# DarylFernandes99/custom-yolo-implmentation

Hardware: AMD Instinct MI355X
Metric: images/sec (640x640 bf16) (higher is better)
Workload: dtype bf16; 1 GPU; preset s (width 32..512, depth 1) 640x640 train step (fwd+DFL/QFL loss+bwd+grad sync+AdamW), COCO-80 synthetic, 32 img/GPU; global_batch=32, parallelism=dp1, hip_graph=True, optimizer_in_graph=True, deterministic_mode=False

## Files before the change

custom-yolo-implmentation_amd/csrc/conv_generic.hip:

```cpp
#include "conv_host.h"

namespace {

template <typename T, int V, bool ACC>
__global__ void k_conv_generic(ConvGeom g, const T* __restrict__ src, const T* __restrict__ wm,
                               const float* __restrict__ bias, T* __restrict__ dst) {
    long total = (long)g.N * g.Hg * g.Wg * g.Cd;
    for (long i = blockIdx.x * (long)blockDim.x + threadIdx.x; i < total; i += (long)gridDim.x * blockDim.x) {
        int cd = (int)(i % g.Cd);
        long q = i / g.Cd;
        int b = (int)(q % g.Wg);
        long t2 = q / g.Wg;
        int a = (int)(t2 % g.Hg);
        long n = t2 / g.Hg;
        float acc = bias ? bias[cd] : 0.f;
        const T* wrow = wm + (long)cd * g.Kpad;
        for (int t = 0; t < g.ntaps; ++t) {
            int hs = a * g.sstride + g.dh[t], ws = b * g.sstride + g.dw[t];
            if (hs < 0 || hs >= g.Hs || ws < 0 || ws >= g.Ws) continue;
            const T* sp = src + ((n * g.Hs + hs) * g.Ws + ws) * (long)g.lds;
            const T* wp = wrow + t * g.Cs;
            for (int c = 0; c < g.Cs; c += V) {
                float xs[V], wv[V];
                load_pack<T, V>(sp + c, xs);
// ... 314 lines not shown
    if (!conv_supported(k, stride)) return 0;
    const int Kpad = round_up32(k * k * Cin);
    if (wgrad_path(x, ldx, dy, ldy, N, H, W, Cin, OH, OW, Cout, dtype, algo) == 2)
        return mfma_wgrad2_ws_elems(Kpad, N, H, W, Cin, OH, OW, Cout, k);
    return (long)Cout * Kpad;
}

int yolo_conv2d_wgrad(const void* x, int ldx, const void* dy, int ldy, float* ws, void* dw_oihw, int dw_dtype, int N,
                      int H, int W, int Cin, int OH, int OW, int Cout, int k, int stride, int dtype, int algo,
                      hipStream_t st) {
    if (!conv_supported(k, stride)) return YOLO_ERR_ARG;
    const int K = k * k * Cin, Kpad = round_up32(K);
    const int path = wgrad_path(x, ldx, dy, ldy, N, H, W, Cin, OH, OW, Cout, dtype, algo);
    if (path == 2)
        return mfma_wgrad2_launch(x, ldx, dy, ldy, ws, dw_oihw, dw_dtype, Kpad, N, H, W, Cin, OH, OW, Cout, k, stride, dtype, st);
    if (algo == 2) return YOLO_ERR_ARG;
    float* dwp = ws;
    int rc = yolo_zero_async(dwp, (size_t)Cout * Kpad * sizeof(float), st);
    if (rc) return rc;
    if (path == 3) {
        rc = mfma_wgrad_launch(x, ldx, dy, ldy, dwp, Kpad, N, H, W, Cin, OH, OW, Cout, k, stride, dtype, st);
    } else if (dtype == YOLO_F32 && f32_wgrad_eligible(x, ldx, dy, ldy, Cin, Cout)) {
        rc = f32_wgrad_launch((const float*)x, ldx, (const float*)dy, ldy, dwp, Kpad, N, H, W, Cin, OH, OW, Cout, k, stride, st);
    } else {
        long nrows = (long)N * OH;
        long elems = (long)Cout * K;
        int gx = (int)((elems + 255) / 256);
        long want_slabs = 4096 / (gx > 0 ? gx : 1);
        if (want_slabs < 1) want_slabs = 1;
        if (want_slabs > nrows) want_slabs = nrows;
        if (want_slabs < 1) want_slabs = 1;
        int rps = (int)((nrows + want_slabs - 1) / want_slabs);
        if (rps < 1) rps = 1;
        int gy = (int)((nrows + rps - 1) / rps);
        if (gy > 0)
            YOLO_DISPATCH_T(dtype, hipLaunchKernelGGL((k_wgrad_generic<T>), dim3(gx, gy), dim3(256), 0, st, (const T*)x, ldx,
                                                      (const T*)dy, ldy, dwp, Kpad, N, H, W, Cin, OH, OW, Cout, k, stride, rps));
        rc = YOLO_LAUNCH_CHECK();
    }
    if (rc) return rc;
    return yolo_conv_unpack_wgrad(dwp, Cout, Cin, k, dw_oihw, dw_dtype, st);
}

}

static dim3 dw_grid(int nrows, int cv) {
    int tpr = cv < 256 ? cv : 256;
    return dim3((unsigned)(nrows < 4096 ? nrows : 4096), (unsigned)ceil_div(cv, tpr));
}

template <bool FLIP>
static int dw_launch(const void* x, int ldx, const float* w, void* y, int ldy, int N, int H, int W, int C, int dtype,
                     int accumulate, hipStream_t st) {
    const int fast = dw_strip_launch(FLIP, x, ldx, w, y, ldy, N, H, W, C, dtype, accumulate, nullptr, st);
    if (fast >= 0) return fast;
    YOLO_DISPATCH_T(dtype, {
        if (vecok<T>(x, ldx, C) && vecok<T>(y, ldy, C)) {
            constexpr int V = vec_of<T>::N;
            hipLaunchKernelGGL((k_dw3x3<T, V, FLIP>), dw_grid(N * H, C / V), dim3(256), 0, st, (const T*)x, ldx, w, (T*)y,
                               ldy, N, H, W, C, accumulate);
        } else {
            hipLaunchKernelGGL((k_dw3x3<T, 1, FLIP>), dw_grid(N * H, C), dim3(256), 0, st, (const T*)x, ldx, w, (T*)y, ldy,
                               N, H, W, C, accumulate);
        }
    });
    return YOLO_LAUNCH_CHECK();
}

extern "C" {

int yolo_dwconv3x3_fwd(const void* x, int ldx, const float* w, void* y, int ldy, int N, int H, int W, int C, int dtype,
                       hipStream_t st) {
    return dw_launch<false>(x, ldx, w, y, ldy, N, H, W, C, dtype, 0, st);
}

int yolo_dwconv3x3_fwd_stats(const void* x, int ldx, const float* w, void* y, int ldy, float* stats, int N, int H, int W, int C,
                             int dtype, hipStream_t st) {
    const int fast = dw_strip_launch(false, x, ldx, w, y, ldy, N, H, W, C, dtype, 0, stats, st);
    return fast < 0 ? 1 : fast;
}

int yolo_dwconv3x3_fwd_act(const void* x, int ldx, const float* w, const float* bias, void* y, int ldy, int N, int H, int W, int C,
                           int act, int dtype, hipStream_t st) {
    if (bias == nullptr || (act != 0 && act != 1)) return YOLO_ERR_ARG;
    const int fast = dw_strip_launch(false, x, ldx, w, y, ldy, N, H, W, C, dtype, 0, nullptr, st, bias, act);
    return fast < 0 ? 1 : fast;
}

int yolo_dwconv3x3_dgrad(const void* dy, int lddy, const float* w, void* dx, int lddx, int N, int H, int W, int C,
                         int accumulate, int dtype, hipStream_t st) {
    return dw_launch<true>(dy, lddy, w, dx, lddx, N, H, W, C, dtype, accumulate, st);
}

int yolo_dw_wgrad_nslab(int N, int H) {
    int nrows = N * H;
    int slabs = nrows < 1024 ? nrows : 1024;
    int rps = (nrows + slabs - 1) / slabs;
    return (nrows + rps - 1) / rps;
}

int yolo_dwconv3x3_wgrad(const void* x, int ldx, const void* dy, int ldy, float* dw, float* partial, int N, int H,
                         int W, int C, int dtype, hipStream_t st) {
    int nrows = N * H;
    int slabs = yolo_dw_wgrad_nslab(N, H);
    int rps = (nrows + slabs - 1) / slabs;
    const int fast = dw_strip_wgrad_launch(x, ldx, dy, ldy, partial, slabs, N, H, W, C, dtype, st);
    if (fast > 0) return fast;
    if (fast < 0) YOLO_DISPATCH_T(dtype, {
        if (vecok<T>(x, ldx, C) && vecok<T>(dy, ldy, C)) {
            constexpr int V = vec_of<T>::N;
            int cv = C / V, tpr = cv < 256 ? cv : 256;
            hipLaunchKernelGGL((k_dw3x3_wgrad<T, V>), dim3(slabs, ceil_div(cv, tpr)), dim3(256), 0, st, (const T*)x, ldx,
                               (const T*)dy, ldy, partial, N, H, W, C, rps);
        } else {
            int tpr = C < 256 ? C : 256;
            hipLaunchKernelGGL((k_dw3x3_wgrad<T, 1>), dim3(slabs, ceil_div(C, tpr)), dim3(256), 0, st, (const T*)x, ldx,
                               (const T*)dy, ldy, partial, N, H, W, C, rps);
        }
    });
    hipLaunchKernelGGL(k_dw_wgrad_finalize, dim3(ceil_div(C * 9, 32)), dim3(1024), 0, st, partial, slabs, C * 9, dw);
    return YOLO_LAUNCH_CHECK();
}

}
```

custom-yolo-implmentation_amd/csrc/conv_host.h:

```cpp
#pragma once
#include "common.h"
#include "conv_geom.h"

enum ConvKind {
    CONV_NONE = -1,
    CONV_VALU = 0,
    CONV_GATHER = 1,
    CONV_HALO = 2,
    CONV_RING = 3,
    CONV_ROWS = 4,
    CONV_UP2 = 5
};
struct RingTile { int bm, bn, nst, bk; };
struct ConvChoice {
    int kind;
    int joint;
    int variant;
    int bn;
    RingTile ring;
};
ConvChoice conv_select(const ConvGeom* gs, int n, int cls, int dtype, const void* src, const void* wm, const void* dst, int algo);

ConvTune& conv_tune();
int conv_wide_flag();

int mfma_conv_addressable(const ConvGeom& g, int dtype, const void* src, const void* wm, const void* dst);

int valu_conv_launch(const ConvGeom& g, const void* src, const void* wm, const float* bias, void* dst, int accumulate, int dtype,
                     hipStream_t st);
int mfma_conv_eligible(const ConvGeom& g, int dtype, const void* src, const void* wm, const void* dst);
int mfma_conv_launch(const ConvGeom& g, int bn, const void* src, const void* wm, const float* bias, void* dst, int accumulate,
                     int dtype, hipStream_t st);
int halo_conv_eligible(const ConvGeom& g);
int halo_conv_launch(const ConvGeom& g, int variant, const void* src, const void* wm, const float* bias, void* dst,
                     int accumulate, int dtype, hipStream_t st);
int ring_conv_eligible(const ConvGeom& g, int dtype, const void* src, const void* wm, const void* dst);
int ring_conv_launch(const ConvGeom* gs, int n, const RingTile& t, const long* wm_off, long wm_elems, const void* src,
                     const void* wm, const float* bias, void* dst, int accumulate, int dtype, hipStream_t st);
int rows_conv_eligible(const ConvGeom& g);
int rows_conv_launch(const ConvGeom& g, int variant, const void* src, const void* wm, const float* bias, void* dst, int accumulate,
                     int dtype, hipStream_t st);
int up2_conv_eligible(const ConvGeom* gs, int dtype);
int up2_conv_launch(const ConvGeom* gs, int variant, const long* wm_off, long wm_elems, const void* src, const void* wm, void* dst,
                    int accumulate, int dtype, hipStream_t st);
int f32_conv_eligible(const ConvGeom& g, const void* src, const void* wm, const void* dst);
int f32_conv_launch(const ConvGeom& g, const float* src, const float* wm, const float* bias, float* dst, int accumulate,
                    hipStream_t st);

int f32_wgrad_eligible(const void* x, int ldx, const void* dy, int ldy, int Cin, int Cout);
int f32_wgrad_launch(const float* x, int ldx, const float* dy, int ldy, float* dwp, int Kpad, int N, int H, int W, int Cin,
                     int OH, int OW, int Cout, int k, int stride, hipStream_t st);
int mfma_wgrad_eligible(int Cin, int Cout, int ldx, int ldy, int dtype, const void* x, const void* dy);
int mfma_wgrad_launch(const void* x, int ldx, const void* dy, int ldy, float* dwp, int Kpad, int N, int H, int W,
                      int Cin, int OH, int OW, int Cout, int k, int stride, int dtype, hipStream_t st);
long mfma_wgrad2_plan(int Kpad, int N, int H, int W, int Cin, int OH, int OW, int Cout, int k);
long mfma_wgrad2_ws_elems(int Kpad, int N, int H, int W, int Cin, int OH, int OW, int Cout, int k);
int mfma_wgrad2_launch(const void* x, int ldx, const void* dy, int ldy, float* part, void* dw_oihw, int dw_dtype, int Kpad,
                       int N, int H, int W, int Cin, int OH, int OW, int Cout, int k, int stride, int dtype, hipStream_t st);

int dw_strip_launch(bool flip, const void* x, int ldx, const float* w, void* y, int ldy, int N, int H, int W, int C, int dtype,
                    int accumulate, float* stats, hipStream_t st, const float* bias = nullptr, int act = 0);
int dw_strip_wgrad_launch(const void* x, int ldx, const void* dy, int ldy, float* partial, int nslab, int N, int H, int W, int C,
                          int dtype, hipStream_t st);

extern "C" int yolo_bn_stats_acc(const void* y, int ldy, long npix, int C, int dtype, float* acc, hipStream_t st);
extern "C" int yolo_copy_channels(const void* src, int ld_src, void* dst, int ld_dst, long npix, int C, int accumulate, int dtype,
                                  hipStream_t st);

static inline bool conv_supported(int k, int stride) { return (k == 1 && stride == 1) || (k == 3 && (stride == 1 || stride == 2)); }
```

custom-yolo-implmentation_amd/csrc/dwconv.hip:

```cpp
#include "conv_host.h"

namespace {

typedef unsigned int u32x4 __attribute__((ext_vector_type(4)));
typedef _Float16 h16x2 __attribute__((ext_vector_type(2)));

template <typename T> __device__ __forceinline__ void unpack8(const u32x4& v, float (&o)[8]);
template <> __device__ __forceinline__ void unpack8<bf16_t>(const u32x4& v, float (&o)[8]) {
#pragma unroll
    for (int i = 0; i < 4; ++i) {
        o[2 * i] = __uint_as_float(v[i] << 16);
        o[2 * i + 1] = __uint_as_float(v[i] & 0xffff0000u);
    }
}
template <> __device__ __forceinline__ void unpack8<f16_t>(const u32x4& v, float (&o)[8]) {
#pragma unroll
    for (int i = 0; i < 4; ++i) {
        const unsigned int u = v[i];
        o[2 * i] = (float)__builtin_bit_cast(_Float16, (unsigned short)(u & 0xffffu));
        o[2 * i + 1] = (float)__builtin_bit_cast(_Float16, (unsigned short)(u >> 16));
    }
}

struct DwGeom {
    int N, H, W, C, ldx, ldy;
    int cvb;
    int ncol;
    int nsh;
    int ncb;
    long total;
    const float* bias;
    int act;
};

constexpr int OOB = (int)0x80000000;

template <bool FLIP>
__device__ __forceinline__ void stage_taps(float* wl, const float* __restrict__ w, int c0, int C, int cvb) {
    for (int i = threadIdx.x; i < cvb * 8 * 9; i += 256) {
        const int ch = i / 9, t = i - ch * 9;
        const float v = (c0 + ch < C) ? w[(long)(c0 + ch) * 9 + (FLIP ? 8 - t : t)] : 0.f;
        wl[((t * 2 + ((ch >> 2) & 1)) * cvb + (ch >> 3)) * 4 + (ch & 3)] = v;
    }
}

template <typename T, int R, bool FLIP>
__global__ __launch_bounds__(256) void k_dw3x3_strip(DwGeom g, const T* __restrict__ x, const float* __restrict__ w,
                                                     T* __restrict__ y, int accumulate, float* __restrict__ stats) {
    extern __shared__ __attribute__((aligned(16))) float wl[];
    const int c0 = blockIdx.y * g.cvb * 8;
    stage_taps<FLIP>(wl, w, c0, g.C, g.cvb);
    __syncthreads();
    const int cgl = threadIdx.x % g.cvb, col = threadIdx.x / g.cvb;
    const int ch = c0 + cgl * 8;
    const bool active = col < g.ncol && ch < g.C;
    float ssum[8], ssq[8];
#pragma unroll
    for (int j = 0; j < 8; ++j) ssum[j] = ssq[j] = 0.f;
    const __amdgpu_buffer_rsrc_t rs =
        __builtin_amdgcn_make_buffer_rsrc(const_cast<T*>(x), 0, g.N * g.H * g.W * g.ldx * 2, 0x00020000);
    const float4* wq = reinterpret_cast<const float4*>(wl) + cgl;
    for (long s = blockIdx.x; active && s < g.total; s += gridDim.x) {
        const int cbk = (int)(s % g.ncb);
        const long t2 = s / g.ncb;
        const int sh = (int)(t2 % g.nsh), n = (int)(t2 / g.nsh);
        const int h0 = sh * R, wc = cbk * g.ncol + col;
        if (wc >= g.W) continue;
        u32x4 v[R + 2][3];
#pragma unroll
        for (int r = 0; r < R + 2; ++r) {
            const int hs = h0 - 1 + r;
            const bool rok = (unsigned)hs < (unsigned)g.H;
#pragma unroll
            for (int c = 0; c < 3; ++c) {
                const int ws = wc - 1 + c;
                const bool ok = rok && (unsigned)ws < (unsigned)g.W;
                const int off = ok ? ((((n * g.H + hs) * g.W + ws) * g.ldx + ch) * 2) : OOB;
                v[r][c] = __builtin_amdgcn_raw_buffer_load_b128(rs, off, 0, 0);
            }
        }
        float acc[R][8];
#pragma unroll
        for (int o = 0; o < R; ++o)
#pragma unroll
            for (int j = 0; j < 8; ++j) acc[o][j] = 0.f;
#pragma unroll
        for (int r = 0; r < R + 2; ++r)
#pragma unroll
            for (int c = 0; c < 3; ++c) {
                float f[8];
                unpack8<T>(v[r][c], f);
#pragma unroll
                for (int kh = 0; kh < 3; ++kh) {
                    const int o = r - kh;
                    if (o < 0 || o >= R) continue;
// ... 78 lines not shown
            if (wc >= g.W) continue;
            u32x4 gv[R], v[R + 2][3];
#pragma unroll
            for (int o = 0; o < R; ++o) {
                const bool ok = h0 + o < g.H;
                gv[o] = __builtin_amdgcn_raw_buffer_load_b128(rsy, ok ? ((((n * g.H + h0 + o) * g.W + wc) * g.ldy + ch) * 2) : OOB, 0, 0);
            }
#pragma unroll
            for (int r = 0; r < R + 2; ++r) {
                const int hs = h0 - 1 + r;
                const bool rok = (unsigned)hs < (unsigned)g.H;
#pragma unroll
                for (int c = 0; c < 3; ++c) {
                    const int ws = wc - 1 + c;
                    const bool ok = rok && (unsigned)ws < (unsigned)g.W;
                    v[r][c] = __builtin_amdgcn_raw_buffer_load_b128(rsx, ok ? ((((n * g.H + hs) * g.W + ws) * g.ldx + ch) * 2) : OOB, 0, 0);
                }
            }
            float gf[R][8];
#pragma unroll
            for (int o = 0; o < R; ++o) unpack8<T>(gv[o], gf[o]);
#pragma unroll
            for (int r = 0; r < R + 2; ++r)
#pragma unroll
                for (int c = 0; c < 3; ++c) {
                    float f[8];
                    unpack8<T>(v[r][c], f);
#pragma unroll
                    for (int kh = 0; kh < 3; ++kh) {
                        const int o = r - kh;
                        if (o < 0 || o >= R) continue;
#pragma unroll
                        for (int j = 0; j < 8; ++j) acc[kh * 3 + c][j] = fmaf(gf[o][j], f[j], acc[kh * 3 + c][j]);
                    }
                }
        }
    }
    float* pw = part + (long)blockIdx.x * g.C * 9;
#pragma unroll
    for (int t = 0; t < 9; ++t) {
        __syncthreads();
#pragma unroll
        for (int j = 0; j < 8; ++j) red[threadIdx.x][j] = active ? acc[t][j] : 0.f;
        __syncthreads();
        for (int o = threadIdx.x; o < g.cvb * 8; o += 256) {
            const int cl = o >> 3, j = o & 7;
            float s = 0.f;
            for (int cc = 0; cc < g.ncol; ++cc) s += red[cc * g.cvb + cl][j];
            if (c0 + o < g.C) pw[(long)(c0 + o) * 9 + t] = s;
        }
    }
}

bool dw_geom(DwGeom& g, const void* x, int ldx, const void* y, int ldy, int N, int H, int W, int C, int R) {
    if (C % 8 || ldx % 8 || ldy % 8 || (reinterpret_cast<uintptr_t>(x) & 15) || (reinterpret_cast<uintptr_t>(y) & 15)) return false;
    if ((long)N * H * W * ldx * 2 >= (1L << 31) || (long)N * H * W * ldy * 2 >= (1L << 31)) return false;
    g.N = N; g.H = H; g.W = W; g.C = C; g.ldx = ldx; g.ldy = ldy;
    const int cv = C / 8;
    g.cvb = cv < 256 ? cv : 256;
    g.ncol = 256 / g.cvb;
    if (g.ncol > W) g.ncol = W;
    g.nsh = (H + R - 1) / R;
    g.ncb = (W + g.ncol - 1) / g.ncol;
    g.total = (long)N * g.nsh * g.ncb;
    g.bias = nullptr; g.act = 0;
    return g.total > 0;
}

}

int dw_strip_launch(bool flip, const void* x, int ldx, const float* w, void* y, int ldy, int N, int H, int W, int C, int dtype,
                    int accumulate, float* stats, hipStream_t st, const float* bias, int act) {
    if (dtype != YOLO_BF16 && dtype != YOLO_F16) return -1;
    constexpr int R = 4;
    DwGeom g;
    if (!dw_geom(g, x, ldx, y, ldy, N, H, W, C, R)) return -1;
    if (bias != nullptr && (flip || stats != nullptr || (reinterpret_cast<uintptr_t>(bias) & 15))) return -1;
    g.bias = bias; g.act = act;
    const dim3 grid((unsigned)(g.total < 4096 ? g.total : 4096), (unsigned)ceil_div(C / 8, g.cvb));
    const size_t lds = (size_t)g.cvb * 8 * 9 * sizeof(float);
#define DW_GO(T_, FLIP_) hipLaunchKernelGGL((k_dw3x3_strip<T_, R, FLIP_>), grid, dim3(256), lds, st, g, (const T_*)x, w, (T_*)y, accumulate, stats)
    if (dtype == YOLO_BF16) { if (flip) DW_GO(bf16_t, true); else DW_GO(bf16_t, false); }
    else { if (flip) DW_GO(f16_t, true); else DW_GO(f16_t, false); }
#undef DW_GO
    return YOLO_LAUNCH_CHECK();
}

int dw_strip_wgrad_launch(const void* x, int ldx, const void* dy, int ldy, float* partial, int nslab, int N, int H, int W, int C,
                          int dtype, hipStream_t st) {
    if (dtype != YOLO_BF16 && dtype != YOLO_F16) return -1;
    constexpr int R = 2;
    DwGeom g;
    if (!dw_geom(g, x, ldx, dy, ldy, N, H, W, C, R)) return -1;
    const dim3 grid((unsigned)nslab, (unsigned)ceil_div(C / 8, g.cvb));
    if (dtype == YOLO_BF16)
        hipLaunchKernelGGL((k_dw3x3_wgrad_strip<bf16_t, R>), grid, dim3(256), 0, st, g, (const bf16_t*)x, (const bf16_t*)dy, partial);
    else
        hipLaunchKernelGGL((k_dw3x3_wgrad_strip<f16_t, R>), grid, dim3(256), 0, st, g, (const f16_t*)x, (const f16_t*)dy, partial);
    return YOLO_LAUNCH_CHECK();
}
```

include/yolo_hip.h:

```cpp
#ifndef YOLO_HIP_H
#define YOLO_HIP_H
#include <stddef.h>
#include <stdint.h>

#ifdef __cplusplus
extern "C" {
#endif

#ifndef __HIP__
typedef struct ihipStream_t* hipStream_t;
#endif

#define YOLO_F32 0
#define YOLO_BF16 1
#define YOLO_F16 2
#define YOLO_ERR_ARG 1001
#define YOLO_ERR_DTYPE 1002
#define YOLO_ACT_IDENTITY 0
#define YOLO_ACT_SILU 1

long yolo_abi_hash(void);

int yolo_memset0(void* p, size_t bytes, hipStream_t st);
int yolo_ncm_to_nhwc(const void* src, int src_dtype, long sn, long sc, long off, void* dst, int dst_dtype, int ld, int N, int C, int HW, hipStream_t st);
// ... 5 lines not shown

int yolo_conv_kpad(int O, int I, int k, int stride, int mode, int cls);
long yolo_conv_dgrad_wbuf_elems(int O, int I, int k, int stride);
int yolo_conv_pack_weights(const void* w_oihw, int w_dtype, int O, int I, int k, int stride, int mode, void* out, int out_dtype, hipStream_t st);
int yolo_conv_unpack_wgrad(const float* dwp, int O, int I, int k, void* dw_oihw, int dw_dtype, hipStream_t st);
int yolo_pack_job_bytes();
int yolo_pack_job_count(int stride, int mode);
long yolo_pack_job_fill(void* jobs_host, const void* w, int w_dtype, void* out, int out_elem_bytes, int O, int I, int k, int stride, int mode, long start);
long yolo_pack_jobs_finalize(void* jobs_host, int njobs);
int yolo_pack_batched(const void* jobs_dev, int njobs, long nchunks, int out_dtype, hipStream_t st);
int yolo_adamw_job_bytes();
int yolo_adamw_job_fill(void* jobs_host, int index, void* p, int p_dtype, const void* g, int g_dtype, float* m, float* v, long n);
long yolo_adamw_jobs_finalize(void* jobs_host, int njobs);
int yolo_adamw_jobs_set_grads(void* jobs_host, int njobs, const void* const* grads);
int yolo_adamw_step(const void* jobs_dev, int njobs, long nchunks, const double* hyper, float* step, const float* grad_scale, const float* found_inf, hipStream_t st);
int yolo_adamw_job_set_ema(void* jobs_host, int index, float* ema, double* ema_ctl);
int yolo_ema_lerp(const void* jobs_dev, int njobs, long nchunks, const double* ema_ctl, const float* skip_flag, hipStream_t st);
int yolo_adamw_amp_step(const void* jobs_dev, int njobs, long nchunks, const double* hyper, float* step, float* amp_state, int* growth_tracker, float growth_factor, float backoff_factor, int growth_interval, hipStream_t st);
int yolo_grad_sqnorm(const void* jobs_dev, int njobs, long nchunks, float* partials, float* found_inf, hipStream_t st);
int yolo_grad_clip_finalize(const float* partials, long nparts, float* clip_state, const float* grad_scale, hipStream_t st);
int yolo_adamw_clip_step(const void* jobs_dev, int njobs, long nchunks, const double* hyper, float* step, const float* grad_scale, const float* found_inf, const float* clip_state, hipStream_t st);
int yolo_amp_update_scale(float* amp_state, int* growth_tracker, float growth_factor, float backoff_factor, int growth_interval, hipStream_t st);
int yolo_sgd_step(const void* jobs_dev, int njobs, long nchunks, const double* hyper, float* step, const float* grad_scale, const float* found_inf, const float* clip_state, hipStream_t st);
int yolo_sgd_amp_step(const void* jobs_dev, int njobs, long nchunks, const double* hyper, float* step, float* amp_state, int* growth_tracker, float growth_factor, float backoff_factor, int growth_interval, hipStream_t st);
int yolo_copy_job_bytes();
int yolo_copy_job_fill(void* jobs_host, int index, const void* src, int src_dtype, void* dst, int dst_dtype, long n);
long yolo_copy_jobs_finalize(void* jobs_host, int njobs);
int yolo_multi_copy(const void* jobs_dev, int njobs, long nchunks, float scale, hipStream_t st);
int yolo_conv2d_fwd(const void* x, int ldx, const void* wp, const float* bias, void* y, int ldy, float* stats_acc, int N, int H, int W, int Cin, int OH, int OW, int Cout, int k, int stride, int dtype, int algo, hipStream_t st);
int yolo_conv2d_fwd_act(const void* x, int ldx, const void* wp, const float* bias, const void* res, int ldr, void* y, int ldy, int N, int H, int W, int Cin, int OH, int OW, int Cout, int k, int stride, int act, int dtype, hipStream_t st);
int yolo_conv2d_dgrad(const void* dy, int lddy, const void* wb, void* dx, int lddx, int N, int H, int W, int Cin, int OH, int OW, int Cout, int k, int stride, int accumulate, int dtype, int algo, hipStream_t st);
int yolo_conv2d_dgrad_acc2(const void* dy, int lddy, const void* wb, void* dx, int lddx, const void* acc2, int ld2, int N, int H, int W, int Cin, int OH, int OW, int Cout, int k, int stride, int dtype, int algo, hipStream_t st);
long yolo_conv2d_wgrad_ws_elems(const void* x, int ldx, const void* dy, int ldy, int N, int H, int W, int Cin, int OH, int OW, int Cout, int k, int stride, int dtype, int algo);
int yolo_conv2d_wgrad(const void* x, int ldx, const void* dy, int ldy, float* ws, void* dw_oihw, int dw_dtype, int N, int H, int W, int Cin, int OH, int OW, int Cout, int k, int stride, int dtype, int algo, hipStream_t st);
int yolo_conv_tune_set(int bn, int tap_inner, int halo, int dma, int ring, int bm, int nst, int bk);
int yolo_wgrad_tune_set(int to, int ti, int blocks, int min_per);
int yolo_wgrad_tune_pf(int pf);
int yolo_conv_wide_set(int on);
int yolo_conv2d_plan(int N, int H, int W, int Cin, int OH, int OW, int Cout, int k, int stride, int mode, int cls, int dtype);
long yolo_conv2d_wgrad_plan(int N, int H, int W, int Cin, int OH, int OW, int Cout, int k, int stride, int dtype);
int yolo_stem_im2col(const void* img, int img_dtype, void* col, int col_dtype, int N, int H, int W, int OH, int OW, hipStream_t st);
int yolo_stem_pack_weights(const void* w, int w_dtype, int Cout, void* out, int out_dtype, hipStream_t st);
int yolo_stem_unpack_wgrad(const float* dw32, int Cout, void* dw, int dw_dtype, hipStream_t st);
int yolo_stem_conv_eligible(int img_dtype, int dtype, int Cout);
int yolo_stem_conv_fwd(const float* img, const void* wp, void* y, int ldy, float* stats, int N, int H, int W, int OH, int OW, int Cout, const float* bias, int act, int dtype, hipStream_t st);
int yolo_stem_wgrad_slabs();
int yolo_stem_wgrad(const float* img, const void* dy, int ldy, float* partial, void* dw, int dw_dtype, int N, int H, int W, int OH, int OW, int Cout, int dtype, hipStream_t st);
int yolo_dwconv3x3_fwd(const void* x, int ldx, const float* w, void* y, int ldy, int N, int H, int W, int C, int dtype, hipStream_t st);
int yolo_dwconv3x3_fwd_stats(const void* x, int ldx, const float* w, void* y, int ldy, float* stats, int N, int H, int W, int C, int dtype, hipStream_t st);
int yolo_dwconv3x3_fwd_act(const void* x, int ldx, const float* w, const float* bias, void* y, int ldy, int N, int H, int W, int C, int act, int dtype, hipStream_t st);
int yolo_dwconv3x3_dgrad(const void* dy, int lddy, const float* w, void* dx, int lddx, int N, int H, int W, int C, int accumulate, int dtype, hipStream_t st);
int yolo_dw_wgrad_nslab(int N, int H);
int yolo_dwconv3x3_wgrad(const void* x, int ldx, const void* dy, int ldy, float* dw, float* partial, int N, int H, int W, int C, int dtype, hipStream_t st);

int yolo_reduce_nblk(long npix, int C);
int yolo_bn_stats(const void* y, int ldy, long npix, int C, int dtype, float* partial, int nblk, hipStream_t st);
int yolo_bn_finalize(const float* partial, int nblk, long count, int C, const void* gamma, const void* beta, void* running_mean, void* running_var, float momentum, float eps, float* mean, float* invstd, float* scale, float* shift, int pdtype, int bdtype, hipStream_t st);
int yolo_bn_eval_coeffs(const void* gamma, const void* beta, const void* running_mean, const void* running_var, float eps, int C, float* scale, float* shift, int pdtype, int bdtype, hipStream_t st);
int yolo_sum_finalize(const float* partial, int nblk, int C, float* out, hipStream_t st);
int yolo_bn_act_fwd(const void* y, int ldy, const float* scale, const float* shift, const void* res, int ldres, void* out, int ldout, long npix, int C, int act, int dtype, hipStream_t st);
int yolo_bn_act_bwd_reduce(const void* dout, int ldd, const void* y, int ldy, const float* scale, const float* shift, const float* mean, const float* invstd, long npix, int C, int act, int dtype, float* partial, int nblk, hipStream_t st);
int yolo_bn_bwd_finalize(const float* partial, int nblk, long count, int C, const void* gamma, const float* mean, const float* invstd, void* dgamma, void* dbeta, float* coef, int pdtype, hipStream_t st);
int yolo_bn_act_bwd_apply(const void* dout, int ldd, const void* y, int ldy, const float* scale, const float* shift, const float* mean, const float* invstd, const float* coef, void* dy, int lddy, long npix, int C, int act, int dtype, hipStream_t st);
int yolo_bn_acc_elems(int C);
int yolo_bn_stats_acc(const void* y, int ldy, long npix, int C, int dtype, float* acc, hipStream_t st);
int yolo_bn_finalize_acc(const float* acc, long count, int C, const void* gamma, const void* beta, void* running_mean, void* running_var, float momentum, float eps, float* mean, float* invstd, float* scale, float* shift, int pdtype, int bdtype, hipStream_t st);
int yolo_bn_act_fwd_train(const void* y, int ldy, const float* acc, long count, const void* gamma, const void* beta, void* running_mean, void* running_var, float momentum, float eps, float* mean, float* invstd, float* scale, float* shift, const void* res, int ldres, void* out, int ldout, long npix, int C, int act, int dtype, int pdtype, int bdtype, hipStream_t st);
int yolo_bn_bwd_reduce_acc(const void* dout, int ldd, const void* y, int ldy, const float* scale, const float* shift, long npix, int C, int act, int dtype, float* acc, hipStream_t st);
int yolo_bn_act_bwd_apply_train(const void* dout, int ldd, const void* y, int ldy, const float* scale, const float* shift, const void* gamma, const float* mean, const float* invstd, const float* acc, long count, void* dgamma, void* dbeta, void* dy, int lddy, long npix, int C, int act, int dtype, int pdtype, hipStream_t st);

int yolo_maxpool5_fwd(const void* x, int ldx, void* out, int ldo, uint8_t* idx, int N, int H, int W, int C, int dtype, hipStream_t st);
int yolo_maxpool5_bwd(const void* dout, int ldd, const uint8_t* idx, void* dx, int ldx, int N, int H, int W, int C, int accumulate, int dtype, hipStream_t st);
int yolo_upsample2x_fwd(const void* x, int ldx, void* out, int ldo, int N, int H, int W, int C, int dtype, hipStream_t st);
int yolo_upsample2x_bwd(const void* dout, int ldd, void* dx, int ldx, int N, int H, int W, int C, int accumulate, int dtype, hipStream_t st);

size_t yolo_attn_stash_bytes(int N, int T_, int heads, int dtype);
size_t yolo_attn_workspace_bytes(int N, int T_, int heads, int dtype);
size_t yolo_attn_stash_bytes_for(int N, int T, int heads, int dk, int dh, int dtype);
size_t yolo_attn_workspace_bytes_for(int N, int T, int heads, int dk, int dh, int dtype);
int yolo_attn_fwd(const void* qkv, int ldq, void* o, int ldo, void* vp, int ldv, void* stash, void* ws, int N, int T_, int heads, int dk, int dh, float scale, int dtype, hipStream_t st);
int yolo_attn_fwd_nograd(const void* qkv, int ldq, void* o, int ldo, void* vp, int ldv, int N, int T_, int heads, int dk, int dh, float scale, int dtype, hipStream_t st);
int yolo_attn_bwd(const void* qkv, int ldq, const void* o, int ldo, const void* d_o, int lddo, const void* d_vp, int lddv, const void* stash, void* ws, void* dqkv, int lddq, int N, int T_, int heads, int dk, int dh, float scale, int dtype, hipStream_t st);

size_t yolo_loss_workspace_bytes(int N, int A, int G);
int yolo_loss_dfl_qfl(const void* preds, const void* anchors, const void* strides, int dtype, int N, int nc, int A, const float* gt, const int* gt_off, const int* gt_img, int G, float lambda_dfl, float lambda_cls, void* dpreds, float* out, void* workspace, const float* grad_scale, hipStream_t st);

int yolo_bbox_iou(const float* box1, const float* box2, int M, float* iou, const float* g, float* db1, float* db2, hipStream_t st);
int yolo_quality_focal_loss(const float* pred, const float* target, int M, int C, float beta, float* out, const float* g, float* dpred, float* dtarget, hipStream_t st);
int yolo_distribution_focal_loss(const float* pred_dist, const float* target_val, int M, int C, float* out, const float* g, float* dpred, float* dtarget, hipStream_t st);

int yolo_head_decode(const void* preds, const void* anchors, const void* strides, void* y, int N, int nc, int A, int dtype, hipStream_t st);
int yolo_dfl_expect(const void* x, void* y, int B, int A, int dtype, hipStream_t st);
int yolo_nms_capacity(int M, int nc, int multi_label);
size_t yolo_nms_workspace_bytes(int bs, int M, int nc, int multi_label);
int yolo_nms(const void* y, int dtype, int bs, int nc, int M, float conf_thres, float iou_thres, const int* classes, int n_classes, int agnostic, int multi_label, int max_det, float* out, int* out_count, int* status, void* workspace, hipStream_t st);

size_t yolo_val_workspace_bytes(int N, int M, int top_k);
int yolo_val_select(const void* y, int dtype, int N, int nc, int M, float conf, int top_k, float* out, int* out_count, void* workspace, hipStream_t st);
int yolo_val_match(const float* pred, const int* count, int N, int top_k, const float* gt, const int* gt_off, double iou_thr, int nc, int skip_empty_gt, long long* counters, int* status, hipStream_t st);

int yolo_prep_image_bytes();
int yolo_prep_image_fill(void* table_host, int index, long off, int H, int W, int flip, int o0, int o1, int o2, int o3, float brightness, float contrast, float saturation, float hue);
int yolo_image_prep(const void* src, const void* table_dev, int N, int S, int jitter, void* stage, float* means, void* out, int out_dtype, float m0, float m1, float m2, float s0, float s1, float s2, hipStream_t st);
int yolo_mosaic_tile_bytes();
int yolo_mosaic_tile_fill(void* table_host, int image, int tile, long off, int H, int W, int flip, int tw, int th, int x0, int y0, int cx, int cy);
int yolo_image_prep_mosaic(const void* src, const void* tiles_dev, const void* table_dev, int N, int S, int fill, int jitter, void* stage, float* means, void* out, int out_dtype, float m0, float m1, float m2, float s0, float s1, float s2, hipStream_t st);
// ... 14 lines not shown
```

Before: 3088 images/s.

## Add row-streaming depthwise 3x3 kernels with planned column tiling and prefetch

Adds new depthwise 3x3 forward/dgrad and wgrad kernels that walk down rows of a column band. They keep a sliding window of input rows in registers, with software prefetch through buffer loads, so neighbouring rows are reused instead of reloaded. A host-side planner picks column count, band height and grid size to limit idle lanes and give enough blocks. The new path is used for large tensors and all wgrad, with an environment variable to force either kernel. Wgrad now writes fewer partial slabs, which shrinks the finalize reduction, at the cost of higher register pressure and more complex code.

Measured after the change: 3123 images/s (median of 6 runs). 1.01x the previous value.

```diff
diff --git a/custom-yolo-implmentation_amd/csrc/conv_generic.hip b/custom-yolo-implmentation_amd/csrc/conv_generic.hip
--- a/custom-yolo-implmentation_amd/csrc/conv_generic.hip
+++ b/custom-yolo-implmentation_amd/csrc/conv_generic.hip
@@ -390,7 +390,7 @@
 template <bool FLIP>
 static int dw_launch(const void* x, int ldx, const float* w, void* y, int ldy, int N, int H, int W, int C, int dtype,
                      int accumulate, hipStream_t st) {
-    const int fast = dw_strip_launch(FLIP, x, ldx, w, y, ldy, N, H, W, C, dtype, accumulate, nullptr, st);
+    const int fast = dw16_launch(FLIP, x, ldx, w, y, ldy, N, H, W, C, dtype, accumulate, nullptr, st);
     if (fast >= 0) return fast;
     YOLO_DISPATCH_T(dtype, {
         if (vecok<T>(x, ldx, C) && vecok<T>(y, ldy, C)) {
@@ -414,14 +414,14 @@
 
 int yolo_dwconv3x3_fwd_stats(const void* x, int ldx, const float* w, void* y, int ldy, float* stats, int N, int H, int W, int C,
                              int dtype, hipStream_t st) {
-    const int fast = dw_strip_launch(false, x, ldx, w, y, ldy, N, H, W, C, dtype, 0, stats, st);
+    const int fast = dw16_launch(false, x, ldx, w, y, ldy, N, H, W, C, dtype, 0, stats, st);
     return fast < 0 ? 1 : fast;
 }
 
 int yolo_dwconv3x3_fwd_act(const void* x, int ldx, const float* w, const float* bias, void* y, int ldy, int N, int H, int W, int C,
                            int act, int dtype, hipStream_t st) {
     if (bias == nullptr || (act != 0 && act != 1)) return YOLO_ERR_ARG;
-    const int fast = dw_strip_launch(false, x, ldx, w, y, ldy, N, H, W, C, dtype, 0, nullptr, st, bias, act);
+    const int fast = dw16_launch(false, x, ldx, w, y, ldy, N, H, W, C, dtype, 0, nullptr, st, bias, act);
     return fast < 0 ? 1 : fast;
 }
 
@@ -442,7 +442,8 @@
     int nrows = N * H;
     int slabs = yolo_dw_wgrad_nslab(N, H);
     int rps = (nrows + slabs - 1) / slabs;
-    const int fast = dw_strip_wgrad_launch(x, ldx, dy, ldy, partial, slabs, N, H, W, C, dtype, st);
+    int nparts = slabs;
+    const int fast = dw16_wgrad_launch(x, ldx, dy, ldy, partial, slabs, &nparts, N, H, W, C, dtype, st);
     if (fast > 0) return fast;
     if (fast < 0) YOLO_DISPATCH_T(dtype, {
         if (vecok<T>(x, ldx, C) && vecok<T>(dy, ldy, C)) {
@@ -456,8 +457,32 @@
                                (const T*)dy, ldy, partial, N, H, W, C, rps);
         }
     });
-    hipLaunchKernelGGL(k_dw_wgrad_finalize, dim3(ceil_div(C * 9, 32)), dim3(1024), 0, st, partial, slabs, C * 9, dw);
+    hipLaunchKernelGGL(k_dw_wgrad_finalize, dim3(ceil_div(C * 9, 32)), dim3(1024), 0, st, partial, nparts, C * 9, dw);
     return YOLO_LAUNCH_CHECK();
 }
 
-}
+int yolo_dw_tune_set(int variant) { return dw_tune_set(variant); }
+
+int yolo_dw_plan(int N, int H, int W, int C, int field) {
+    if (N < 1 || H < 1 || W < 1 || C < 1) return -1;
+    if (C % 8 || (long)N * H * W * C * 2 >= (1L << 31)) return 0;
+    if (field == 0 || field == 12) return dw_takes_rows(N, H, W, C, field == 12) ? 1 : 2;
+    const DwPlan p = dw_plan(N, H, W, C);
+    const int nslab = yolo_dw_wgrad_nslab(N, H);
+    switch (field) {
+        case 1: return p.ncol;
+        case 2: return p.ncb;
+        case 3: return p.cvb;
+        case 4: return p.wg;
+        case 5: return p.hb;
+        case 6: return p.nb;
+        case 7: return p.grid;
+        case 8: return p.hb_wg;
+        case 9: return p.nb_wg;
+        case 10: return p.grid_wg < nslab ? p.grid_wg : nslab;
+        case 11: return p.ncy;
+        default: return -1;
+    }
+}
+
+}
diff --git a/custom-yolo-implmentation_amd/csrc/conv_host.h b/custom-yolo-implmentation_amd/csrc/conv_host.h
--- a/custom-yolo-implmentation_amd/csrc/conv_host.h
+++ b/custom-yolo-implmentation_amd/csrc/conv_host.h
@@ -58,10 +58,20 @@
 int mfma_wgrad2_launch(const void* x, int ldx, const void* dy, int ldy, float* part, void* dw_oihw, int dw_dtype, int Kpad,
                        int N, int H, int W, int Cin, int OH, int OW, int Cout, int k, int stride, int dtype, hipStream_t st);
 
-int dw_strip_launch(bool flip, const void* x, int ldx, const float* w, void* y, int ldy, int N, int H, int W, int C, int dtype,
-                    int accumulate, float* stats, hipStream_t st, const float* bias = nullptr, int act = 0);
-int dw_strip_wgrad_launch(const void* x, int ldx, const void* dy, int ldy, float* partial, int nslab, int N, int H, int W, int C,
-                          int dtype, hipStream_t st);
+struct DwPlan {
+    int cvb, ncy;
+    int ncol, ncb;
+    int wg;
+    int hb, nb, grid;
+    int hb_wg, nb_wg, grid_wg;
+};
+DwPlan dw_plan(int N, int H, int W, int C);
+int dw_tune_set(int variant);
+bool dw_takes_rows(int N, int H, int W, int C, bool wgrad);
+int dw16_launch(bool flip, const void* x, int ldx, const float* w, void* y, int ldy, int N, int H, int W, int C, int dtype,
+                int accumulate, float* stats, hipStream_t st, const float* bias = nullptr, int act = 0);
+int dw16_wgrad_launch(const void* x, int ldx, const void* dy, int ldy, float* partial, int nslab, int* nrows, int N, int H, int W,
+                      int C, int dtype, hipStream_t st);
 
 extern "C" int yolo_bn_stats_acc(const void* y, int ldy, long npix, int C, int dtype, float* acc, hipStream_t st);
 extern "C" int yolo_copy_channels(const void* src, int ld_src, void* dst, int ld_dst, long npix, int C, int accumulate, int dtype,
diff --git a/custom-yolo-implmentation_amd/csrc/dwconv.hip b/custom-yolo-implmentation_amd/csrc/dwconv.hip
--- a/custom-yolo-implmentation_amd/csrc/dwconv.hip
+++ b/custom-yolo-implmentation_amd/csrc/dwconv.hip
@@ -1,3 +1,5 @@
+#include <cstdlib>
+#include <cstring>
 #include "conv_host.h"
 
 namespace {
@@ -26,6 +28,7 @@
     int N, H, W, C, ldx, ldy;
     int cvb;
     int ncol;
+    int hb;
     int nsh;
     int ncb;
     long total;
@@ -37,10 +40,21 @@
 
 template <bool FLIP>
 __device__ __forceinline__ void stage_taps(float* wl, const float* __restrict__ w, int c0, int C, int cvb) {
-    for (int i = threadIdx.x; i < cvb * 8 * 9; i += 256) {
+    for (int i = threadIdx.x; i < cvb * 8 * 9; i += blockDim.x) {
         const int ch = i / 9, t = i - ch * 9;
         const float v = (c0 + ch < C) ? w[(long)(c0 + ch) * 9 + (FLIP ? 8 - t : t)] : 0.f;
         wl[((t * 2 + ((ch >> 2) & 1)) * cvb + (ch >> 3)) * 4 + (ch & 3)] = v;
+    }
+}
+
+constexpr int DW_TAP_LD = 76;
+constexpr size_t DW_TAP_MAX = 256 * DW_TAP_LD * sizeof(float);
+template <bool FLIP>
+__device__ __forceinline__ void stage_taps_rows(float* wl, const float* __restrict__ w, int c0, int C, int cvb) {
+    for (int i = threadIdx.x; i < cvb * 8 * 9; i += blockDim.x) {
+        const int ch = i / 9, t = i - ch * 9;
+        const float v = (c0 + ch < C) ? w[(long)(c0 + ch) * 9 + (FLIP ? 8 - t : t)] : 0.f;
+        wl[(ch >> 3) * DW_TAP_LD + t * 8 + (ch & 7)] = v;
     }
 }
 
@@ -225,30 +239,327 @@
     }
 }
 
-bool dw_geom(DwGeom& g, const void* x, int ldx, const void* y, int ldy, int N, int H, int W, int C, int R) {
+constexpr int DW_PF = 2;
+constexpr int DW_PF_WGRAD = 1;
+
+struct DwCols { unsigned off[3]; };
+
+__device__ __forceinline__ DwCols dw_cols(int wc, int W, int ld, int ch) {
+    DwCols c;
+#pragma unroll
+    for (int k = 0; k < 3; ++k) {
+        const int ws = wc - 1 + k;
+        c.off[k] = (unsigned)ws < (unsigned)W ? (unsigned)((ws * ld + ch) * 2) : (unsigned)OOB;
+    }
+    return c;
+}
+
+template <typename T>
+__device__ __forceinline__ u32x4 dw_load(const T* p, int bytes, bool rok, unsigned coloff, unsigned rowoff) {
+    const __amdgpu_buffer_rsrc_t rs = __builtin_amdgcn_make_buffer_rsrc(const_cast<T*>(p), 0, rok ? bytes : 0, 0x00020000);
+    return __builtin_amdgcn_raw_buffer_load_b128(rs, (int)coloff, (int)(rok ? rowoff : 0u), 0);
+}
+
+template <typename T>
+__device__ __forceinline__ void dw_load_row(u32x4 (&v)[3], const T* p, int bytes, const DwCols& c, int r, int rmax,
+                                            unsigned rowbytes, unsigned imgoff) {
+    const bool rok = r >= 0 && r <= rmax;
+    const unsigned rb = imgoff + (unsigned)r * rowbytes;
+#pragma unroll
+    for (int k = 0; k < 3; ++k) v[k] = dw_load<T>(p, bytes, rok, c.off[k], rb);
+}
+
+template <typename T, bool FLIP>
+__global__ __launch_bounds__(256, FLIP ? 4 : 3) void k_dw3x3_rows(DwGeom g, const T* __restrict__ x, const float* __restrict__ w,
+                                                    T* __restrict__ y, int accumulate, float* __restrict__ stats) {
+    constexpr int D = DW_PF + 3;
+    extern __shared__ __attribute__((aligned(16))) float wl[];
+    const int c0 = blockIdx.y * g.cvb * 8;
+    stage_taps_rows<FLIP>(wl, w, c0, g.C, g.cvb);
+    __syncthreads();
+    const int cgl = threadIdx.x % g.cvb, col = threadIdx.x / g.cvb;
+    const int ch = c0 + cgl * 8;
+    const bool active = col < g.ncol && ch < g.C;
+    float ssum[8], ssq[8];
+#pragma unroll
+    for (int j = 0; j < 8; ++j) ssum[j] = ssq[j] = 0.f;
+    const int xbytes = g.N * g.H * g.W * g.ldx * 2;
+    const int ybytes = accumulate ? g.N * g.H * g.W * g.ldy * 2 : 0;
+    const float4* wq = reinterpret_cast<const float4*>(wl + cgl * DW_TAP_LD);
+    float4 b0 = make_float4(0.f, 0.f, 0.f, 0.f), b1 = b0;
+    if (!FLIP && g.bias != nullptr && active) {
+        b0 = *reinterpret_cast<const float4*>(g.bias + ch);
+        b1 = *reinterpret_cast<const float4*>(g.bias + ch + 4);
+    }
+    const unsigned xrow = (unsigned)(g.W * g.ldx * 2), yrow = (unsigned)(g.W * g.ldy * 2);
+    for (long s = blockIdx.x; s < g.total; s += gridDim.x) {
+        const int cbk = (int)(s % g.ncb);
+        const long t2 = s / g.ncb;
+        const int sh = (int)(t2 % g.nsh), n = (int)(t2 / g.nsh);
+        const int h0 = sh * g.hb, wc = cbk * g.ncol + col;
+        if (!active || wc >= g.W) continue;
+        const int h1 = h0 + g.hb < g.H ? h0 + g.hb : g.H;
+        const int nr = h1 - h0, rmax = h1 < g.H ? h1 : g.H - 1;
+        const DwCols cx = dw_cols(wc, g.W, g.ldx, ch);
+        const unsigned ximg = (unsigned)n * g.H * xrow, yimg = (unsigned)n * g.H * yrow;
+        const unsigned ycol = (unsigned)((wc * g.ldy + ch) * 2);
+        u32x4 v[D][3], pv[D];
+#pragma unroll
+        for (int i = 0; i < D - 1; ++i) dw_load_row<T>(v[i], x, xbytes, cx, h0 - 1 + i, rmax, xrow, ximg);
+        pv[0] = dw_load<T>(y, ybytes, true, ycol, yimg + (unsigned)h0 * yrow);
+        for (int jb = 0; jb < nr; jb += D) {
+#pragma unroll
+            for (int u = 0; u < D; ++u) {
+                const int h = h0 + jb + u;
+                if (h >= h1) break;
+                asm volatile("" ::: "memory");
+                pv[(u + 1) % D] = dw_load<T>(y, ybytes, h + 1 < h1, ycol, yimg + (unsigned)(h + 1) * yrow);
+                dw_load_row<T>(v[(u + D - 1) % D], x, xbytes, cx, h + 1 + DW_PF, rmax, xrow, ximg);
+                float acc[8];
+#pragma unroll
+                for (int j = 0; j < 8; ++j) acc[j] = 0.f;
+#pragma unroll
+                for (int kh = 0; kh < 3; ++kh)
+#pragma unroll
+                    for (int c = 0; c < 3; ++c) {
+                        float f[8];
+                        asm volatile("" : "+v"(v[(u + kh) % D][c]));
+                        unpack8<T>(v[(u + kh) % D][c], f);
+                        const float4 w0 = wq[(kh * 3 + c) * 2], w1 = wq[(kh * 3 + c) * 2 + 1];
+                        acc[0] = fmaf(f[0], w0.x, acc[0]); acc[1] = fmaf(f[1], w0.y, acc[1]);
+                        acc[2] = fmaf(f[2], w0.z, acc[2]); acc[3] = fmaf(f[3], w0.w, acc[3]);
+                        acc[4] = fmaf(f[4], w1.x, acc[4]); acc[5] = fmaf(f[5], w1.y, acc[5]);
+                        acc[6] = fmaf(f[6], w1.z, acc[6]); acc[7] = fmaf(f[7], w1.w, acc[7]);
+                    }
+                T* dst = y + ((long)(n * g.H + h) * g.W + wc) * g.ldy + ch;
+                if (!FLIP && g.bias != nullptr) {
+                    acc[0] += b0.x; acc[1] += b0.y; acc[2] += b0.z; acc[3] += b0.w;
+                    acc[4] += b1.x; acc[5] += b1.y; acc[6] += b1.z; acc[7] += b1.w;
+                    if (g.act) {
+#pragma unroll
+                        for (int j = 0; j < 8; ++j) acc[j] = acc[j] * __frcp_rn(1.f + __expf(-acc[j]));
+                    }
+                }
+                if (accumulate) {
+                    float prev[8];
+                    unpack8<T>(pv[u % D], prev);
+#pragma unroll
+                    for (int j = 0; j < 8; ++j) acc[j] += prev[j];
+                }
+                store_pack<T, 8>(dst, acc);
+                if (!FLIP && stats != nullptr) {
+#pragma unroll
+                    for (int j = 0; j < 8; ++j) {
+                        const float r2 = to_f<T>(from_f<T>(acc[j]));
+                        ssum[j] += r2;
+                        ssq[j] += r2 * r2;
+                    }
+                }
+            }
+        }
+    }
+    if (FLIP || stats == nullptr) return;
+    __shared__ float red[256][9];
+    float* o = stats + (long)(blockIdx.x & 7) * 2 * g.C;
+#pragma unroll
+    for (int pass = 0; pass < 2; ++pass) {
+        __syncthreads();
+#pragma unroll
+        for (int j = 0; j < 8; ++j) red[threadIdx.x][j] = active ? (pass ? ssq[j] : ssum[j]) : 0.f;
+        __syncthreads();
+        for (int e = threadIdx.x; e < g.cvb * 8; e += blockDim.x) {
+            const int cl = e >> 3, j = e & 7;
+            float t = 0.f;
+            for (int cc = 0; cc < g.ncol; ++cc) t += red[cc * g.cvb + cl][j];
+            if (c0 + e < g.C) atomicAdd(o + pass * g.C + c0 + e, t);
+        }
+    }
+}
+
+constexpr int DW_RED_LD = 73;
+constexpr size_t DW_RED_MAX = 256 * DW_RED_LD * sizeof(float);
+
+template <typename T>
+__global__ __launch_bounds__(256, 3) void k_dw3x3_wgrad_rows(DwGeom g, const T* __restrict__ x, const T* __restrict__ dy,
+                                                          float* __restrict__ part) {
+    constexpr int D = DW_PF_WGRAD + 3;
+    extern __shared__ __attribute__((aligned(16))) float red[];
+    const int c0 = blockIdx.y * g.cvb * 8;
+    const int cgl = threadIdx.x % g.cvb, col = threadIdx.x / g.cvb;
+    const int ch = c0 + cgl * 8;
+    const bool active = col < g.ncol && ch < g.C;
+    float acc[9][8];
+#pragma unroll
+    for (int t = 0; t < 9; ++t)
+#pragma unroll
+        for (int j = 0; j < 8; ++j) acc[t][j] = 0.f;
+    const int xbytes = g.N * g.H * g.W * g.ldx * 2, ybytes = g.N * g.H * g.W * g.ldy * 2;
+    const unsigned xrow = (unsigned)(g.W * g.ldx * 2), yrow = (unsigned)(g.W * g.ldy * 2);
+    for (long s = blockIdx.x; s < g.total; s += gridDim.x) {
+        const int cbk = (int)(s % g.ncb);
+        const long t2 = s / g.ncb;
+        const int sh = (int)(t2 % g.nsh), n = (int)(t2 / g.nsh);
+        const int h0 = sh * g.hb, wc = cbk * g.ncol + col;
+        if (!active || wc >= g.W) continue;
+        const int h1 = h0 + g.hb < g.H ? h0 + g.hb : g.H;
+        const int nr = h1 - h0, rmax = h1 < g.H ? h1 : g.H - 1;
+        const DwCols cx = dw_cols(wc, g.W, g.ldx, ch);
+        const unsigned ximg = (unsigned)n * g.H * xrow, yimg = (unsigned)n * g.H * yrow;
+        const unsigned ycol = (unsigned)((wc * g.ldy + ch) * 2);
+        u32x4 v[D][3], gv[D];
+#pragma unroll
+        for (int i = 0; i < D - 1; ++i) dw_load_row<T>(v[i], x, xbytes, cx, h0 - 1 + i, rmax, xrow, ximg);
+#pragma unroll
+        for (int i = 0; i <= DW_PF_WGRAD; ++i) gv[i] = dw_load<T>(dy, ybytes, h0 + i < h1, ycol, yimg + (unsigned)(h0 + i) * yrow);
+        for (int jb = 0; jb < nr; jb += D) {
+#pragma unroll
+            for (int u = 0; u < D; ++u) {
+                const int h = h0 + jb + u;
+                if (h >= h1) break;
+                const int hn = h + 1 + DW_PF_WGRAD;
+                gv[(u + 1 + DW_PF_WGRAD) % D] = dw_load<T>(dy, ybytes, hn < h1, ycol, yimg + (unsigned)hn * yrow);
+                dw_load_row<T>(v[(u + D - 1) % D], x, xbytes, cx, hn, rmax, xrow, ximg);
+                float gf[8];
+                unpack8<T>(gv[u % D], gf);
+#pragma unroll
+                for (int kh = 0; kh < 3; ++kh)
+#pragma unroll
+                    for (int c = 0; c < 3; ++c) {
+                        float f[8];
+                        asm volatile("" : "+v"(v[(u + kh) % D][c]));
+                        unpack8<T>(v[(u + kh) % D][c], f);
+#pragma unroll
+                        for (int j = 0; j < 8; ++j) acc[kh * 3 + c][j] = fmaf(gf[j], f[j], acc[kh * 3 + c][j]);
+                    }
+            }
+        }
+    }
+    const int nthr = g.cvb * g.ncol;
+    if ((int)threadIdx.x < nthr) {
+#pragma unroll
+        for (int t = 0; t < 9; ++t)
+#pragma unroll
+            for (int j = 0; j < 8; ++j) red[threadIdx.x * DW_RED_LD + t * 8 + j] = acc[t][j];
+    }
+    __syncthreads();
+    float* pw = part + (long)blockIdx.x * g.C * 9;
+    for (int o = threadIdx.x; o < g.cvb * 72; o += blockDim.x) {
+        const int cl = o / 72, k = o - cl * 72;
+        float sum = 0.f;
+        for (int cc = 0; cc < g.ncol; ++cc) sum += red[(cc * g.cvb + cl) * DW_RED_LD + k];
+        const int c = c0 + cl * 8 + (k & 7);
+        if (c < g.C) pw[(long)c * 9 + (k >> 3)] = sum;
+    }
+}
+
+bool dw_eligible(const void* x, int ldx, const void* y, int ldy, int N, int H, int W, int C) {
     if (C % 8 || ldx % 8 || ldy % 8 || (reinterpret_cast<uintptr_t>(x) & 15) || (reinterpret_cast<uintptr_t>(y) & 15)) return false;
     if ((long)N * H * W * ldx * 2 >= (1L << 31) || (long)N * H * W * ldy * 2 >= (1L << 31)) return false;
+    return (long)N * H * W > 0;
+}
+
+void dw_geom(DwGeom& g, int ldx, int ldy, int N, int H, int W, int C, int R) {
     g.N = N; g.H = H; g.W = W; g.C = C; g.ldx = ldx; g.ldy = ldy;
     const int cv = C / 8;
     g.cvb = cv < 256 ? cv : 256;
     g.ncol = 256 / g.cvb;
     if (g.ncol > W) g.ncol = W;
+    g.hb = R;
     g.nsh = (H + R - 1) / R;
     g.ncb = (W + g.ncol - 1) / g.ncol;
     g.total = (long)N * g.nsh * g.ncb;
     g.bias = nullptr; g.act = 0;
-    return g.total > 0;
-}
-
-}
-
-int dw_strip_launch(bool flip, const void* x, int ldx, const float* w, void* y, int ldy, int N, int H, int W, int C, int dtype,
-                    int accumulate, float* stats, hipStream_t st, const float* bias, int act) {
+}
+
+int& dw_variant() {
+    static int v = [] {
+        const char* e = getenv("YOLO_DW_KERNEL");
+        return e == nullptr ? 0 : strcmp(e, "strip") == 0 ? 1 : strcmp(e, "rows") == 0 ? 2 : 0;
+    }();
+    return v;
+}
+
+}
+
+DwPlan dw_plan(int N, int H, int W, int C) {
+    DwPlan p{};
+    const int cv = C / 8;
+    p.cvb = cv < 256 ? cv : 256;
+    p.ncy = ceil_div(cv, p.cvb);
+    const int maxcol = 256 / p.cvb < W ? 256 / p.cvb : W;
+    long best = -1;
+    for (int nc = 1; nc <= maxcol; ++nc) {
+        const int ncb = (W + nc - 1) / nc, idle = ncb * nc - W;
+        if (4 * idle > ncb * nc) continue;
+        const long cost = (long)ncb * (nc + 2) * 1024 + idle;
+        if (best < 0 || cost <= best) { best = cost; p.ncol = nc; p.ncb = ncb; }
+    }
+    p.wg = (p.cvb * p.ncol + 63) / 64 * 64;
+    const long per_band = (long)N * p.ncb * p.ncy;
+    const int hmin = H < 4 ? H : 4;
+    const long want = (512 + per_band - 1) / per_band;
+    p.hb = (int)(H / want) > hmin ? (int)(H / want) : hmin;
+    p.nb = (H + p.hb - 1) / p.hb;
+    const long most = 512 / per_band > 1 ? 512 / per_band : 1;
+    p.hb_wg = (int)((H + most - 1) / most) > hmin ? (int)((H + most - 1) / most) : hmin;
+    p.nb_wg = (H + p.hb_wg - 1) / p.hb_wg;
+    const long items = (long)N * p.ncb * p.nb, items_wg = (long)N * p.ncb * p.nb_wg;
+    p.grid = (int)(items < 1024 ? items : 1024);
+    p.grid_wg = (int)(items_wg < 512 ? items_wg : 512);
+    return p;
+}
+
+int dw_tune_set(int variant) {
+    if (variant < 0 || variant > 2) return YOLO_ERR_ARG;
+    dw_variant() = variant;
+    return YOLO_OK;
+}
+
+bool dw_takes_rows(int N, int H, int W, int C, bool wgrad) {
+    const int v = dw_variant();
+    if (v != 0) return v == 2;
+    return wgrad || (long)N * H * W * C * 2 >= (16L << 20);
+}
+
+namespace {
+
+void dw_rows_geom(DwGeom& g, const DwPlan& p, int ldx, int ldy, int N, int H, int W, int C, bool wgrad) {
+    g.N = N; g.H = H; g.W = W; g.C = C; g.ldx = ldx; g.ldy = ldy;
+    g.cvb = p.cvb; g.ncol = p.ncol; g.ncb = p.ncb;
+    g.hb = wgrad ? p.hb_wg : p.hb;
+    g.nsh = wgrad ? p.nb_wg : p.nb;
+    g.total = (long)N * g.nsh * g.ncb;
+    g.bias = nullptr; g.act = 0;
+}
+
+}
+
+int dw16_launch(bool flip, const void* x, int ldx, const float* w, void* y, int ldy, int N, int H, int W, int C, int dtype,
+                int accumulate, float* stats, hipStream_t st, const float* bias, int act) {
     if (dtype != YOLO_BF16 && dtype != YOLO_F16) return -1;
+    if (!dw_eligible(x, ldx, y, ldy, N, H, W, C)) return -1;
+    if (bias != nullptr && (flip || stats != nullptr || (reinterpret_cast<uintptr_t>(bias) & 15))) return -1;
+    DwGeom g;
+    if (dw_takes_rows(N, H, W, C, false)) {
+        const DwPlan p = dw_plan(N, H, W, C);
+        dw_rows_geom(g, p, ldx, ldy, N, H, W, C, false);
+        g.bias = bias; g.act = act;
+        const dim3 grid((unsigned)p.grid, (unsigned)p.ncy);
+        const size_t lds = (size_t)g.cvb * DW_TAP_LD * sizeof(float);
+        static unsigned long long done[4] = {0, 0, 0, 0};
+#define DW_GO(T_, FLIP_)                                                                                                        \
+    do {                                                                                                                        \
+        if (int rc = yolo_allow_dyn_lds(reinterpret_cast<const void*>(&k_dw3x3_rows<T_, FLIP_>), DW_TAP_MAX,                    \
+                                        done[(dtype == YOLO_BF16 ? 0 : 2) + (FLIP_ ? 1 : 0)])) return rc;                       \
+        hipLaunchKernelGGL((k_dw3x3_rows<T_, FLIP_>), grid, dim3(p.wg), lds, st, g, (const T_*)x, w, (T_*)y, accumulate, stats); \
+    } while (0)
+        if (dtype == YOLO_BF16) { if (flip) DW_GO(bf16_t, true); else DW_GO(bf16_t, false); }
+        else { if (flip) DW_GO(f16_t, true); else DW_GO(f16_t, false); }
+#undef DW_GO
+        return YOLO_LAUNCH_CHECK();
+    }
     constexpr int R = 4;
-    DwGeom g;
-    if (!dw_geom(g, x, ldx, y, ldy, N, H, W, C, R)) return -1;
-    if (bias != nullptr && (flip || stats != nullptr || (reinterpret_cast<uintptr_t>(bias) & 15))) return -1;
+    dw_geom(g, ldx, ldy, N, H, W, C, R);
     g.bias = bias; g.act = act;
     const dim3 grid((unsigned)(g.total < 4096 ? g.total : 4096), (unsigned)ceil_div(C / 8, g.cvb));
     const size_t lds = (size_t)g.cvb * 8 * 9 * sizeof(float);
@@ -259,12 +570,30 @@
     return YOLO_LAUNCH_CHECK();
 }
 
-int dw_strip_wgrad_launch(const void* x, int ldx, const void* dy, int ldy, float* partial, int nslab, int N, int H, int W, int C,
-                          int dtype, hipStream_t st) {
+int dw16_wgrad_launch(const void* x, int ldx, const void* dy, int ldy, float* partial, int nslab, int* nrows, int N, int H, int W,
+                      int C, int dtype, hipStream_t st) {
     if (dtype != YOLO_BF16 && dtype != YOLO_F16) return -1;
+    if (!dw_eligible(x, ldx, dy, ldy, N, H, W, C)) return -1;
+    DwGeom g;
+    if (dw_takes_rows(N, H, W, C, true)) {
+        const DwPlan p = dw_plan(N, H, W, C);
+        dw_rows_geom(g, p, ldx, ldy, N, H, W, C, true);
+        *nrows = p.grid_wg < nslab ? p.grid_wg : nslab;
+        const dim3 grid((unsigned)*nrows, (unsigned)p.ncy);
+        const size_t lds = (size_t)g.cvb * g.ncol * DW_RED_LD * sizeof(float);
+        static unsigned long long done_bf16 = 0, done_f16 = 0;
+        if (dtype == YOLO_BF16) {
+            if (int rc = yolo_allow_dyn_lds(reinterpret_cast<const void*>(&k_dw3x3_wgrad_rows<bf16_t>), DW_RED_MAX, done_bf16)) return rc;
+            hipLaunchKernelGGL((k_dw3x3_wgrad_rows<bf16_t>), grid, dim3(p.wg), lds, st, g, (const bf16_t*)x, (const bf16_t*)dy, partial);
+        } else {
+            if (int rc = yolo_allow_dyn_lds(reinterpret_cast<const void*>(&k_dw3x3_wgrad_rows<f16_t>), DW_RED_MAX, done_f16)) return rc;
+            hipLaunchKernelGGL((k_dw3x3_wgrad_rows<f16_t>), grid, dim3(p.wg), lds, st, g, (const f16_t*)x, (const f16_t*)dy, partial);
+        }
+        return YOLO_LAUNCH_CHECK();
+    }
     constexpr int R = 2;
-    DwGeom g;
-    if (!dw_geom(g, x, ldx, dy, ldy, N, H, W, C, R)) return -1;
+    dw_geom(g, ldx, ldy, N, H, W, C, R);
+    *nrows = nslab;
     const dim3 grid((unsigned)nslab, (unsigned)ceil_div(C / 8, g.cvb));
     if (dtype == YOLO_BF16)
         hipLaunchKernelGGL((k_dw3x3_wgrad_strip<bf16_t, R>), grid, dim3(256), 0, st, g, (const bf16_t*)x, (const bf16_t*)dy, partial);
diff --git a/include/yolo_hip.h b/include/yolo_hip.h
--- a/include/yolo_hip.h
+++ b/include/yolo_hip.h
@@ -81,6 +81,8 @@
 int yolo_dwconv3x3_dgrad(const void* dy, int lddy, const float* w, void* dx, int lddx, int N, int H, int W, int C, int accumulate, int dtype, hipStream_t st);
 int yolo_dw_wgrad_nslab(int N, int H);
 int yolo_dwconv3x3_wgrad(const void* x, int ldx, const void* dy, int ldy, float* dw, float* partial, int N, int H, int W, int C, int dtype, hipStream_t st);
+int yolo_dw_tune_set(int variant);
+int yolo_dw_plan(int N, int H, int W, int C, int field);
 
 int yolo_reduce_nblk(long npix, int C);
 int yolo_bn_stats(const void* y, int ldy, long npix, int C, int dtype, float* partial, int nblk, hipStream_t st);
```
